# fperezgamonal/flownet2-tf

Measured on AMD Instinct MI355X. Metric: forward pairs/sec at 512x384 (FlowNet2), higher is better.
Workload: dtype f16x2 (split fp16 hi+lo operands, 3 fp16 MFMAs per product, fp32 accumulate); 1 GPU; FlowNet2 forward, batch=4 synthetic 512x384 pairs per GPU, seeded synthetic weights; pairs_per_gpu=4, parallelism=dp1 (no collective)

## Files before the change

### flownet2-tf_amd/csrc/conv.hip

```cpp
#include "conv_common.h"
#include <cstdlib>

namespace fn2 {

template <typename T, typename OutT, int TC, int WC, int WP>
__global__ void __launch_bounds__(256) conv_igemm_kernel(const ConvArgs p) {
  constexpr int CH = 16 / (int)sizeof(T);
  constexpr int BC = WC * TC * 16;
  constexpr int BP = WP * 64;
  constexpr int NT = 256;
  static_assert(WC * WP == 4, "4 waves per block");
  constexpr int NPR = BP / 64;
  constexpr int NWR = (BC * 4 + NT - 1) / NT;
  constexpr int WSWZ_BIT = (TC == 4) ? 5 : (TC == 2) ? 4 : 3;
  __shared__ uint4 lds[2][(BC + BP) * 4];

  const int tid = threadIdx.x, lane = tid & 63, wave = tid >> 6;
  const int wc = wave / WP, wp = wave % WP;
  const int cid = tid & 3;

  int pad_y = p.pad, pad_x = p.pad, oy_off = 0, ox_off = 0, osc = 1;
  const T* wgt = reinterpret_cast<const T*>(p.wgt);
  const int phase = blockIdx.z / p.splitk, split = blockIdx.z - phase * p.splitk;
  if (p.deconv) {
// ... 840 lines not shown
  FN2_REQUIRE(d->up_src == nullptr || ((d->kind == 1 || d->kind == 5) && d->up_w != nullptr && d->up_c0 >= 0 &&
                                       d->up_c0 + 2 <= d->out.cs && !d->accumulate),
              "conv2d: up_src rides on a kind-1 / kind-5 transposed conv (up_w set, [up_c0, up_c0 + 2) inside the out buffer)");
  FN2_REQUIRE(d->cin_pad % 8 == 0 && d->cin_pad >= d->in.c, "conv2d: cin_pad must be a multiple of 8 >= Cin");
  FN2_REQUIRE(d->in.cs % 8 == 0 && d->in.c0 % 8 == 0, "conv2d: input channel stride/offset must be multiples of 8");
  if (d->kind != 2)
    FN2_REQUIRE(d->in.c0 + d->cin_pad <= d->in.cs, "conv2d: padded input channels exceed the buffer stride");
  const int esz = dtype_size(d->in.dtype);
  const int CH = 16 / esz;
  FN2_REQUIRE(d->kpad > 0 && d->kpad % (4 * CH) == 0, "conv2d: kpad must be a multiple of one k-step");
  fn2_conv_plan plan;
  rc = fn2_conv2d_plan(d->in.dtype, d->cin_pad, d->out.c, &plan);
  if (rc) return rc;
  const bool wfrag = d->wgt_layout == 2;
  if (wfrag)
    FN2_REQUIRE(plan.layout == 1 && plan.cout_tile >= 64 && d->in.dtype == FN2_F16X2 && d->kind != 2,
                "conv2d: wgt_layout 2 (fragment order) is for split-fp16 layers with more than 32 output channels");
  else
    FN2_REQUIRE(d->wgt_layout == plan.layout, "conv2d: wgt_layout %d does not match fn2_conv2d_plan (%d)", d->wgt_layout,
                plan.layout);
  const int tile = plan.cout_tile;
  FN2_REQUIRE(d->cout_pad % tile == 0 && d->cout_pad >= d->out.c, "conv2d: cout_pad must be a multiple of the cout tile");
  FN2_REQUIRE(d->act == FN2_ACT_NONE || d->act == FN2_ACT_LEAKY, "conv2d: bad activation");
  FN2_REQUIRE(d->out.dtype == d->in.dtype || d->out.dtype == FN2_F32 ||
                  (d->in.dtype == FN2_F32 && d->out.dtype == FN2_F16X2),
              "conv2d: output dtype must be the input dtype, fp32, or split-fp16 from an fp32 stem");
  if (d->in.dtype == FN2_F16X2) FN2_REQUIRE(d->in.cs % 8 == 0 && d->in.c0 % 8 == 0, "conv2d: split-fp16 views are group (8) aligned");
  if (d->out.dtype == FN2_F16X2) FN2_REQUIRE(d->out.cs % 8 == 0 && d->out.c0 % 8 == 0, "conv2d: split-fp16 views are group (8) aligned");

  ConvArgs& a = *out;
  a = ConvArgs{};
  a.KH_KW_hint = 0;
// ... 16 lines not shown
  } else if (d->kind == 2) {
    FN2_REQUIRE(d->kh >= 1 && d->kw >= 1 && d->stride >= 1 && d->pad == 0, "stem conv: pad must be baked into the input buffer");
    FN2_REQUIRE(d->in.c0 == 0 && d->in.c == d->in.cs, "stem conv: the input view must be the whole buffer");
    FN2_REQUIRE(d->cin_pad >= d->kw * d->in.cs, "stem conv: run (cin_pad) shorter than kw*cs");
    FN2_REQUIRE(d->wgt_layout == 1, "stem conv: runs on the LDS-DMA kernel only (run must be whole 128-byte lines)");
    a.KH = d->kh; a.KW = 1; a.stride = d->stride; a.pad = 0;
    a.KH_KW_hint = d->kw;
    a.OH = (d->in.h - d->kh) / d->stride + 1;
    a.OW = (d->in.w - d->kw) / d->stride + 1;
    FN2_REQUIRE(a.OH >= 1 && a.OW >= 1, "stem conv: kernel does not fit");
    FN2_REQUIRE(d->out.h == a.OH && d->out.w == a.OW, "stem conv: output spatial size %dx%d != expected %dx%d",
                d->out.h, d->out.w, a.OH, a.OW);
    a.deconv = 0; a.ph_pad0 = a.ph_pad1 = 0;
  } else if (d->kind == 5) {
    FN2_REQUIRE(d->kh == 4 && d->kw == 4 && d->stride == 2, "deconv (kind 5): only k=4 s=2 crop 1");
    FN2_REQUIRE((d->out.c == 16 || d->out.c == 32) && d->in.dtype == FN2_F16X2 && d->wgt_layout == 1 && d->cout_pad == 2 * d->out.c,
                "deconv (kind 5): 16 or 32 output channels, split-fp16 input, cout_pad = 2 Cout");
    FN2_REQUIRE(d->in.w % 128 == 0, "deconv (kind 5): input width must be a multiple of 128 (halo kernel tiles)");
    a.KH = 2; a.KW = 3; a.stride = 1; a.pad = 0;
    a.OH = d->in.h; a.OW = d->in.w;
    FN2_REQUIRE(d->out.h == 2 * d->in.h && d->out.w == 2 * d->in.w, "deconv: output must be 2H x 2W");
    a.deconv = 1;
    a.ph_pad0 = 1; a.ph_pad1 = 0;
    phases = 2;
  } else if (d->kind == 1) {
    FN2_REQUIRE(d->kh == 4 && d->kw == 4 && d->stride == 2, "deconv: only k=4 s=2 crop 1 (flownet_s.py:53-63)");
    a.KH = 2; a.KW = 2; a.stride = 1; a.pad = 0;
    a.OH = d->in.h; a.OW = d->in.w;
    FN2_REQUIRE(d->out.h == 2 * d->in.h && d->out.w == 2 * d->in.w, "deconv: output must be 2H x 2W");
    a.deconv = 1;
    a.ph_pad0 = 1; a.ph_pad1 = 0;
// ... 163 lines not shown
    const int kper = cdiv(a.ksteps, sk);
    sk = cdiv(a.ksteps, kper);
    if (d->wgt_layout >= 1) sk = cdiv(a.ksteps / 2, cdiv(kper, 2));
  }
  return sk < 1 ? 1 : sk;
}

int fn2_conv2d_kernel_name(const fn2_conv_desc* d, char* name, int cap) {
  FN2_REQUIRE(name && cap > 0, "conv2d_kernel_name: no buffer");
  name[0] = 0;
  if (!d || d->wgt_layout < 1 || is_flow_head(d)) return FN2_OK;
  conv_name_sink() = ConvNameSink{name, cap};
  const int rc = fn2_conv2d(d, nullptr);
  conv_name_sink() = ConvNameSink{nullptr, 0};
  return rc;
}

int fn2_conv2d(const fn2_conv_desc* d, void* stream) {
  ConvArgs a;
  int tile, phases;
  int rc = build_args(d, &a, &tile, &phases);
  if (rc) return rc;
  hipStream_t s = (hipStream_t)stream;
  if (is_flow_head(d)) {
    int blocks = grid_for((long)a.M * 64, 256);
    if (d->in.dtype == FN2_F16X2 && a.M <= 4096 && !(a.dbg & 32768)) {
      a.dbg |= 16384;
      blocks = a.M;
    } else {
      a.dbg &= ~16384;
// ... 274 lines not shown
```

### flownet2-tf_amd/csrc/conv2.hip

```cpp
#include "conv_common.h"

#include <type_traits>
#include <algorithm>
#include <utility>

#ifndef FN2_X2_ORDER
#define FN2_X2_ORDER 0
#endif
#ifndef FN2_CONV_ABLATE
#define FN2_CONV_ABLATE 0
#endif
#ifndef FN2_SETPRIO
#define FN2_SETPRIO 1
#endif

namespace fn2 {

typedef __attribute__((address_space(3))) void* lptr_t;

constexpr unsigned kOobOffset = 0x80000000u;

typedef int v4i_t __attribute__((ext_vector_type(4)));
typedef unsigned u32x4_t __attribute__((ext_vector_type(4)));

__device__ __forceinline__ v4i_t make_rsrc(const void* base, int bytes) {
  const unsigned long long a = (unsigned long long)base;
  return v4i_t{(int)(a & 0xffffffffu), (int)((a >> 32) & 0xffffu), bytes, 0x00020000};
}

__device__ __forceinline__ void dma16(const v4i_t rsrc, const void* lds, unsigned voff, int soff) {
  const unsigned la = (unsigned)(unsigned long long)(lptr_t)lds;
  asm volatile("s_mov_b32 m0, %0\n\ts_nop 0\n\tbuffer_load_dwordx4 %1, %2, %3 offen lds"
               :: "s"(la), "v"(voff), "s"(rsrc), "s"(soff) : "memory");
}

__device__ __forceinline__ void h5_ring_pixel(const ConvArgs& p, long m) {
  const int lane = threadIdx.x & 63;
  const int H = p.OH, W = p.OW, ring = 2 * W + 2 * (H - 2);
  const int nitems = 25 * p.h5_groups;
  const size_t case_stride = (size_t)nitems * 16;
  const x2_t* in = reinterpret_cast<const x2_t*>(p.in);
  float* pf = reinterpret_cast<float*>(p.out);
  const int n = (int)(m / ring), r = (int)(m - (long)n * ring);
  int y, x;
  if (r < W) { y = 0; x = r; }
  else if (r < 2 * W) { y = H - 1; x = r - W; }
  else { const int q = r - 2 * W; y = 1 + (q >> 1); x = (q & 1) ? W - 1 : 0; }
  const int cy = y == 0 ? 0 : (y == H - 1 ? 2 : 1), cx = x == 0 ? 0 : (x == W - 1 ? 2 : 1);
// ... 195 lines not shown
          dma16(rsrc_w, &lds[(wave * (BC / 4) + i * 8) * 8], woff[i], ((ky * p.KW + kx) * spt + sc) * 128);
      }
    } else {
      constexpr int j = i - NWI;
      const unsigned tbit = (1u << ky) | (1u << (8 + kx));
      const int toff = ((ky * p.W + kx) * p.in_cs + sc * 8 * CH) * ESZ;
      const unsigned voff = ((vmask[j] & tbit) == tbit && wstage < kt1) ? (unsigned)(roff[j] + toff) : kOobOffset;
      if (!(FN2_CONV_ABLATE && (p.dbg & 1)))
        dma16(rsrc_x, &lds[(BOFF + wave * (BP / 4) + j * 8) * 8], voff, 0);
    }
  };
  u32x4_t wfa[WREG ? 4 : 1], wfb[WREG ? 4 : 1], wfc[(WREG && STAGES == 3) ? 4 : 1];
  const unsigned wlane = (unsigned)lane * 16u;
  const int wtile_off = WREG ? ((c0 >> 5) + wc) * (p.ksteps * 4096) : 0;
  auto load_w = [&](u32x4_t (&wf)[WREG ? 4 : 1]) {
    if constexpr (WREG) {
      const int soff = wtile_off + ((ky * p.KW + kx) * spt + sc) * 4096;
      asm volatile("buffer_load_dwordx4 %0, %4, %5, %6 offen\n\t"
                   "buffer_load_dwordx4 %1, %4, %5, %6 offen offset:1024\n\t"
                   "buffer_load_dwordx4 %2, %4, %5, %6 offen offset:2048\n\t"
                   "buffer_load_dwordx4 %3, %4, %5, %6 offen offset:3072"
                   : "=&v"(wf[0]), "=&v"(wf[1]), "=&v"(wf[2]), "=&v"(wf[3])
                   : "v"(wlane), "s"(rsrc_w), "s"(soff) : "memory");
    }
  };
  auto advance1 = [&]() {
    ++wstage;
    if (tap_outer) {
      if (++sc == spt) {
        sc = 0;
        if (++kx == kwi) { kx = 0; ++ky; }
      }
      if (ky == khi) { ky = 0; sc = spt; }
    } else if (++kx == kwi) {
      kx = 0;
      if (++ky == khi) { ky = 0; ++sc; }
    }
  };
  auto advance = [&]() {
// ... 2 lines not shown
  };
  auto issue_stage = [&](uint4* lds) {
    [&]<int... I>(std::integer_sequence<int, I...>) {
      (issue_piece(std::integral_constant<int, I>{}, lds), ...);
    }(std::make_integer_sequence<int, NWI + NPI>{});
    advance();
  };
  auto issue_stage_w = [&](uint4* lds, u32x4_t (&wf)[WREG ? 4 : 1]) {
    [&]<int... I>(std::integer_sequence<int, I...>) {
      (issue_piece(std::integral_constant<int, I>{}, lds), ...);
    }(std::make_integer_sequence<int, NWI + NPI>{});
    load_w(wf);
    advance();
  };
  auto wait_w = [&](u32x4_t (&wf)[WREG ? 4 : 1]) {
    if constexpr (WREG)
      asm volatile("s_waitcnt vmcnt(0)" : "+v"(wf[0]), "+v"(wf[1]), "+v"(wf[2]), "+v"(wf[3]) :: "memory");
  };

  const int fr = lane & 31, fh = lane >> 5, fsw = (fr >> 1) & 7;
  f32x16 acc[TCN][TPN];
#pragma unroll
  for (int tc = 0; tc < TCN; ++tc)
#pragma unroll
    for (int tp = 0; tp < TPN; ++tp)
#pragma unroll
      for (int q = 0; q < 16; ++q) acc[tc][tp][q] = 0.f;
  f32x4 acc16[M16 ? TCN * 2 : 1][M16 ? TPN * 2 : 1];
  if constexpr (M16) {
#pragma unroll
    for (int a = 0; a < TCN * 2; ++a)
#pragma unroll
// ... 452 lines not shown
  }
  if (wide) {
    const int rr = lane / CPR, ch = lane - rr * CPR;
    OutT* ob = out + p.out_c0 + c0 + wc * WCOLS + ch * 4;
#pragma unroll
    for (int i = 0; i < WROWS / RPI; ++i) {
      const int row = i * RPI + rr;
      const uint4 v = *reinterpret_cast<const uint4*>(tl + row * RS + ch * 4);
      const int opix = rowoff[row];
      if (opix >= 0) *reinterpret_cast<uint4*>(ob + (size_t)opix * p.out_cs) = v;
    }
  }
#endif
}

template <typename OutT, int WC, int WP, int TCN, int TPN, int KW>
__global__ void __launch_bounds__(256) conv_halo_kernel(const ConvArgs p) {
#if defined(__HIP_DEVICE_COMPILE__)
  using T = x2_t;
  constexpr int ESZ = 4;
  constexpr int BC = WC * TCN * 32, BP = WP * TPN * 32;
  static_assert(WC * WP == 4, "4 waves per block");
  constexpr int NWI = BC / 32;
  constexpr int BROWS = BP + 8;
  constexpr int NBP = BROWS / 8;
  constexpr int NBW = (NBP + 3) / 4;
  __shared__ uint4 ldsA[2][BC * 8];
  __shared__ uint4 ldsB[2][BROWS * 8];

  const int tid = threadIdx.x, lane = tid & 63;
  const int wave = __builtin_amdgcn_readfirstlane(tid >> 6);
  const int wc = wave / WP, wp = wave % WP;

  int pad_y = p.pad, pad_x = p.pad, oy_off = 0, ox_off = 0, osc = 1;
  const T* wgt = reinterpret_cast<const T*>(p.wgt);
  const int phase = blockIdx.z;
  const unsigned wrow_bytes = (unsigned)p.ksteps * 128u;
  if (p.merged) {
    pad_y = phase ? p.ph_pad1 : p.ph_pad0; pad_x = 1; oy_off = phase; ox_off = 0; osc = 2;
    wgt += (size_t)phase * p.cout_pad * (wrow_bytes / ESZ);
  } else if (p.deconv) {
    const int a = phase >> 1, b = phase & 1;
// ... 23 lines not shown
    const int row = wave * (BC / 4) + j * 8 + lrow;
    woff[j] = (unsigned)(c0 + row) * wrow_bytes + (unsigned)((lphys ^ ((row >> 1) & 7)) * 16);
  }
  int boff[NBW];
  bool bok[NBW];
#pragma unroll
  for (int j = 0; j < NBW; ++j) {
    const int q = wave + 4 * j;
    const int e = q * 8 + lrow;
    const int ix = ix_base + e;
    bok[j] = q < NBP && e < BP + KW - 1 && ix >= 0 && ix < p.W;
    boff[j] = (((tn * p.H + iy_base) * p.W + ix) * p.in_cs + p.in_c0) * ESZ + (lphys ^ ((e >> 1) & 7)) * 16;
  }
  const int spt = p.cin_chunks >> 3;
  const int nsup = spt * p.KH;
  auto issue_B = [&](int sup, uint4* lds) {
    const int sc = sup / p.KH, ky = sup - sc * p.KH;
    const bool yok = (unsigned)(iy_base + ky) < (unsigned)p.H;
    const int toff = (ky * p.W * p.in_cs) * ESZ + sc * 128;
#pragma unroll
    for (int j = 0; j < NBW; ++j) {
      const int q = wave + 4 * j;
      if (q < NBP) dma16(rsrc_x, &lds[q * 64], (bok[j] && yok) ? (unsigned)(boff[j] + toff) : kOobOffset, 0);
    }
  };
  auto issue_A = [&](int sup, int kx, uint4* lds) {
    const int sc = sup / p.KH, ky = sup - sc * p.KH;
    const int soff = ((ky * KW + kx) * spt + sc) * 128;
#pragma unroll
    for (int j = 0; j < NWI; ++j) dma16(rsrc_w, &lds[(wave * (BC / 4) + j * 8) * 8], woff[j], soff);
  };

  const int fr = lane & 31, fh = lane >> 5, fsw = (fr >> 1) & 7;
  f32x16 acc[TCN][TPN];
#pragma unroll
  for (int tc = 0; tc < TCN; ++tc)
#pragma unroll
    for (int tp = 0; tp < TPN; ++tp)
#pragma unroll
// ... 18 lines not shown
      }
#pragma unroll
      for (int tc = 0; tc < TCN; ++tc)
#pragma unroll
        for (int tp = 0; tp < TPN; ++tp) {
          acc[tc][tp] = mfma_32x32x16<f16_t>(al[tc], bh[tp], acc[tc][tp]);
          acc[tc][tp] = mfma_32x32x16<f16_t>(ah[tc], bl[tp], acc[tc][tp]);
          acc[tc][tp] = mfma_32x32x16<f16_t>(ah[tc], bh[tp], acc[tc][tp]);
        }
    }
#if FN2_SETPRIO
    __builtin_amdgcn_s_setprio(0);
#endif
  };

  issue_B(0, ldsB[0]);
  issue_A(0, 0, ldsA[0]);
  asm volatile("s_waitcnt vmcnt(0)" ::: "memory");
  __syncthreads();
  int abuf = 0;
  for (int sup = 0; sup < nsup; ++sup) {
#pragma unroll
    for (int kx = 0; kx < KW; ++kx) {
      if (kx + 1 < KW) issue_A(sup, kx + 1, ldsA[abuf ^ 1]);
      else if (sup + 1 < nsup) issue_A(sup + 1, 0, ldsA[abuf ^ 1]);
      if (kx == 0 && sup + 1 < nsup) issue_B(sup + 1, ldsB[(sup + 1) & 1]);
      compute(ldsA[abuf], ldsB[sup & 1], kx);
      asm volatile("s_waitcnt vmcnt(0)" ::: "memory");
      __syncthreads();
      abuf ^= 1;
    }
  }

  OutT* out = reinterpret_cast<OutT*>(p.out);
  const bool vec16 = (p.out_cs % 8 == 0) && (p.out_c0 % 8 == 0);
  constexpr int ERS = 36;
  static_assert(sizeof(ldsA) >= 4 * 32 * ERS * 4 || sizeof(ldsB) >= 4 * 32 * ERS * 4, "epilogue tiles fit a stage array");
  float* const etl = reinterpret_cast<float*>(sizeof(ldsA) >= 4 * 32 * ERS * 4 ? &ldsA[0][0] : &ldsB[0][0]) + wave * (32 * ERS);
#pragma unroll
  for (int tc = 0; tc < TCN; ++tc) {
    int cout_base = c0 + wc * TCN * 32 + tc * 32 + fh * 16;
    int bsel = 0;
    if (p.merged) { bsel = cout_base / p.Cout; cout_base -= bsel * p.Cout; if (bsel > 1) continue; }
    float bias[16];
#pragma unroll
// ... 510 lines not shown
    snprintf(conv_name_sink().buf, conv_name_sink().cap, "conv_stem_kernel<%s, %d>",
             is_x2<OutT>::value ? "fn2::x2_t" : "float", a.ksteps);
    return true;
  }
  switch (a.ksteps) {
    case 1: hipLaunchKernelGGL((conv_stem_kernel<OutT, 1>), dim3(blocks), dim3(256), 0, s, a, ntiles); break;
    case 2: hipLaunchKernelGGL((conv_stem_kernel<OutT, 2>), dim3(blocks), dim3(256), 0, s, a, ntiles); break;
    case 3: hipLaunchKernelGGL((conv_stem_kernel<OutT, 3>), dim3(blocks), dim3(256), 0, s, a, ntiles); break;
    default: hipLaunchKernelGGL((conv_stem_kernel<OutT, 4>), dim3(blocks), dim3(256), 0, s, a, ntiles); break;
  }
  return true;
}

template <typename OutT>
static bool launch_halo(const ConvArgs& a, int tile, int phases, hipStream_t s) {
  if (((a.dbg & 2048) && !a.merged) || a.stride != 1 || a.splitk != 1 || a.kg != 1 || !a.bp64 || a.wfrag || (a.KW != 2 && a.KW != 3)) return false;
  if (a.deconv && (a.kh_ph[0] != a.KH || a.kh_ph[1] != a.KH || a.kw_ph[0] != a.KW || a.kw_ph[1] != a.KW)) return false;
  if (tile == 128 && a.bp64 == 2 && !(a.dbg & 4096)) return false;
  if (a.bp64 == 3) return false;
  const int bp = tile == 128 ? 64 : 128;
  if (a.OW % bp != 0 || a.M % bp != 0) return false;
  dim3 block(256);
#define FN2_HALO(GY, ...)                                                                         \
  do {                                                                                            \
    dim3 grid(a.M / bp, GY, phases);                                                              \
    if (conv_name_sink().buf)                                                                     \
      snprintf(conv_name_sink().buf, conv_name_sink().cap, "conv_halo_kernel<%s, %s, %d>",       \
               is_x2<OutT>::value ? "fn2::x2_t" : "float", #__VA_ARGS__, a.KW);                    \
    else if (a.KW == 3) hipLaunchKernelGGL((conv_halo_kernel<OutT, __VA_ARGS__, 3>), grid, block, 0, s, a); \
    else hipLaunchKernelGGL((conv_halo_kernel<OutT, __VA_ARGS__, 2>), grid, block, 0, s, a);      \
  } while (0)
  if (tile == 128) FN2_HALO(a.cout_pad / 128, 2, 2, 2, 1);
  else if (tile == 64) FN2_HALO(a.cout_pad / 64, 1, 4, 2, 1);
  else FN2_HALO(a.cout_pad / 32, 1, 4, 1, 1);
#undef FN2_HALO
  return true;
}

template <typename T> static const char* type_name();
template <> const char* type_name<float>() { return "float"; }
template <> const char* type_name<bf16_t>() { return "__bf16"; }
template <> const char* type_name<f16_t>() { return "_Float16"; }
template <> const char* type_name<x2_t>() { return "fn2::x2_t"; }

ConvNameSink& conv_name_sink() {
  static thread_local ConvNameSink sink{nullptr, 0};
  return sink;
}

// ... 4 lines not shown
  const char* e_m16 = getenv("FN2_M16_MIN");
  const bool m16 = is_x2<T>::value && !(a.dbg & 512) &&
                   ((a.dbg & 1024) || (e_m16 && tile == 128 && a.bp64 == 1 && a.kg == 1 && a.splitk == 1 &&
                                       blocks64 >= atoi(e_m16)));
#define FN2_LAUNCH2(GX, GY, THREADS, ...)                                                              \
  do {                                                                                                 \
    dim3 grid(GX, GY, z);                                                                              \
    if (conv_name_sink().buf)                                                                          \
      snprintf(conv_name_sink().buf, conv_name_sink().cap, "conv_igemm2_kernel<%s, %s, %s, %s>", type_name<T>(), \
               type_name<OutT>(), #__VA_ARGS__, m16 ? "true" : "false");                              \
    else if (m16) hipLaunchKernelGGL((conv_igemm2_kernel<T, OutT, __VA_ARGS__, is_x2<T>::value>), grid, dim3(THREADS), 0, s, a); \
    else hipLaunchKernelGGL((conv_igemm2_kernel<T, OutT, __VA_ARGS__, false>), grid, dim3(THREADS), 0, s, a);            \
  } while (0)
  if (a.wfrag) {
    if constexpr (is_x2<T>::value) {
      if (tile == 64) {
        dim3 grid(cdiv(a.M, 128), a.cout_pad / 64, z);
        if (conv_name_sink().buf)
          snprintf(conv_name_sink().buf, conv_name_sink().cap, "conv_igemm2_kernel<%s, %s, 2, 2, 1, 2, 2, 1, false, true, %s>",
                   type_name<T>(), type_name<OutT>(), a.splitk > 1 ? "true" : "false");
        else if (a.splitk > 1)
          hipLaunchKernelGGL((conv_igemm2_kernel<T, OutT, 2, 2, 1, 2, 2, 1, false, true, true>), grid, dim3(256), 0, s, a);
        else
          hipLaunchKernelGGL((conv_igemm2_kernel<T, OutT, 2, 2, 1, 2, 2, 1, false, true, false>), grid, dim3(256), 0, s, a);
      } else {
        dim3 grid(cdiv(a.M, 64), a.cout_pad / 128, z);
        const bool slab = a.splitk > 1;
        ConvArgs ah = a;
        if (a.fh_M > 0 && slab && !conv_name_sink().buf) {
          const char* e = getenv("FN2_FH_BLOCKS");
          const long per_z = (long)grid.x * grid.y;
// ... 89 lines not shown
```

### flownet2-tf_amd/src/_hip.py

```python
import ctypes as C
import os

import numpy as np
import torch

_HERE = os.path.dirname(os.path.abspath(__file__))
LIB_PATH = os.path.join(os.path.dirname(_HERE), "lib", "libflownet2_hip.so")

FN2_F32, FN2_BF16, FN2_F16, FN2_F16X2 = 0, 1, 2, 3
ACT_NONE, ACT_LEAKY = 0, 1
OK = 0
ERR_INVALID_ARGUMENT, ERR_UNSUPPORTED, ERR_HIP = -1, -2, -3


class Fn2Tensor(C.Structure):
    _fields_ = [("data", C.c_void_p), ("dtype", C.c_int32), ("n", C.c_int32), ("h", C.c_int32),
                ("w", C.c_int32), ("c", C.c_int32), ("cs", C.c_int32), ("c0", C.c_int32)]


class Fn2ConvPlan(C.Structure):
    _fields_ = [("layout", C.c_int32), ("cout_tile", C.c_int32), ("kstep_elems", C.c_int32),
                ("wgt_dtype", C.c_int32)]


# ... 28 lines not shown
    "fn2_correlation_f32_ws": (_i, [_p, _p, _p] + [_i] * 9 + [_p, C.c_int64, _p]),
    "fn2_correlation_grad_f32": (_i, [_p] * 5 + [_i] * 9 + [_p]),
    "fn2_flow_warp_f32": (_i, [_p, _p, _p, _i, _i, _i, _i, _p]),
    "fn2_flow_warp_grad_f32": (_i, [_p] * 5 + [_i] * 4 + [_p]),
    "fn2_downsample_f32": (_i, [_p, _p] + [_i] * 6 + [_p]),
    "fn2_downsample_scaled_f32": (_i, [_p, _f, _p] + [_i] * 6 + [_p]),
    "fn2_fill_zero": (_i, [_p, C.c_int64, _p]),
    "fn2_add_f32": (_i, [_p, _p, C.c_int64, _p]),
    "fn2_slice_copy_f32": (_i, [_tp, _p, _p]),
    "fn2_resize_bilinear_f32": (_i, [_p, _p] + [_i] * 6 + [_f, _p]),
    "fn2_conv2d_plan": (_i, [_i, _i, _i, C.POINTER(Fn2ConvPlan)]),
    "fn2_conv2d_workspace_bytes": (C.c_int64, [C.POINTER(Fn2ConvDesc)]),
    "fn2_conv2d": (_i, [C.POINTER(Fn2ConvDesc), _p]),
    "fn2_conv2d_kernel_name": (_i, [C.POINTER(Fn2ConvDesc), C.c_char_p, _i]),
    "fn2_conv2d_splits": (_i, [C.POINTER(Fn2ConvDesc)]),
    "fn2_augment_f32": (_i, [_p, _p, _p, _p, _i, _i, _i, _i, _i, _i, _p]),
    "fn2_flow_augmentation_f32": (_i, [_p, _p, _p, _p, _i, _i, _i, _i, _i, _p]),
    "fn2_flow_head_gather": (_i, [_p, _i, _p, _p, _i, _i, _i, _p]),
    "fn2_upsample_flow": (_i, [_p, _p, _p, _tp, _i, _i, _i, _p]),
    "fn2_flow_head_tail": (_i, [_p, _i, _i, _p, _p, _i, _i, _i, _i, _p, _p, _tp, _p]),
    "fn2_flow_head_tail_slabs": (_i, [_p, _i, _i, C.c_int64, _f, _i, _p, _p, _i, _i, _i, _i, _p, _p, _tp, _p]),
    "fn2_flow_head_ring": (_i, [_tp, _p, _p, _p, _p]),
    "fn2_flow_head5": (_i, [_tp, _p, _i, _i, _f, _p, _p, _i, _p, _p, _p]),
    "fn2_u8_to_f32_lut": (_i, [_p, _p, _p, C.c_int64, _p]),
    "fn2_pack_pair": (_i, [_p, _p, _tp, _i, _p]),
    "fn2_pack_interp_u8": (_i, [_p, _p, _p, _p, _p, _tp, _i, _p]),
    "fn2_pack_image": (_i, [_p, _i, _tp, _i, _i, _p]),
    "fn2_pack_image_s2d": (_i, [_p, _i, _i, _i, _tp, _i, _i, _p]),
    "fn2_correlation_fused": (_i, [_tp, _tp, _tp, _i, _i, _i, _p]),
    "fn2_stack_input": (_i, [_p, _p, _p, _tp, _i, _p]),
# ... 115 lines not shown
```

### flownet2-tf_amd/src/engine.py

```python
import ctypes as C
import math
import os

import numpy as np
import torch

from . import _hip, netdefs, weights as W

_DT = {"f32": torch.float32, "bf16": torch.bfloat16, "f16": torch.float16, "f16x2": torch.float32}
_CODE = {"f32": _hip.FN2_F32, "bf16": _hip.FN2_BF16, "f16": _hip.FN2_F16, "f16x2": _hip.FN2_F16X2}
_TILE_ARGS = {128: "2, 2, 2, 2", 64: "1, 4, 2, 2", 32: "1, 4, 1, 2"}


def conv2_kernel_args(tile, m, cout_pad, phases, x2=True):
    dbg = int(os.environ.get("FN2_CONV_DBG", "0"))
    blocks64 = -(-m // 64) * (cout_pad // 128) * phases if tile == 128 else 0
    big = "FN2_M16_MIN" in os.environ and blocks64 >= max(int(os.environ["FN2_M16_MIN"]), 513)
    m16 = "true" if (x2 and not dbg & 512 and (dbg & 1024 or big)) else "false"
    full = dbg & 32
    if tile < 128:
        base = {64: "1, 4, 2, 2, 2, 1", 32: "1, 4, 1, 2, 2, 1"}[tile] if full else {64: "1, 4, 2, 1, 2, 1", 32: "1, 4, 1, 1, 2, 1"}[tile]
        return f"{base}, {m16}"
    blocks = -(-m // 64) * (cout_pad // 128) * phases
    if not full and int(os.environ.get("FN2_KG", "1")):
# ... 224 lines not shown
                out_scale = 2.0 ** (-k2)
        wdev = W.packed_to_device(packed, plan.wgt_dtype, self.device)
        d = _hip.Fn2ConvDesc()
        d.inp = self._v(sbuf, sc, sc0)
        d.out = self._v(dbuf, dc, dc0)
        d.wgt = wdev.data_ptr()
        d.bias = bias.data_ptr() if bias is not None else None
        d.kind = 0 if kind == "conv" else (5 if merged else 1)
        d.kh = d.kw = k
        d.stride, d.pad = stride, pad
        d.act = _hip.ACT_LEAKY if act else _hip.ACT_NONE
        d.cin_pad, d.cout_pad, d.kpad = cin_pad, cout_pad, kpad
        d.wgt_layout = layout
        d.out_scale = out_scale
        frag = False
        if (self.fragment_weights and layout == 1 and tile >= int(os.environ.get("FN2_WREG_TILE_MIN", "128"))
                and plan.wgt_dtype == _hip.FN2_F16X2 and self._wants_fragments(d)):
            wdev = W.to_fragment_order(wdev)
            d.wgt, d.wgt_layout, frag = wdev.data_ptr(), 2, True
        self.keep += [d, wdev, bias]
        self.conv_descs.append(d)
        self.desc_branch.append(self._branch)
        up_rec = None
        if self._pending_head is not None and kind != "conv":
            hd = self._pending_head
            assert up_after is not None and hd.inp.data == d.inp.data and hd.inp.c0 == d.inp.c0, (scope, name)
            d.head = C.addressof(hd)
            self._pending_head = None
        if up_after is not None:
            assert kind != "conv" and (not merged or cout == 16)
            up_name, up_src, (ubuf, uc0, uc) = up_after
            assert ubuf is dbuf and uc == 2
# ... 35 lines not shown
        need = int(self.lib.fn2_conv2d_workspace_bytes(C.byref(d)))
        if need <= 0 or not int(os.environ.get("FN2_HEAD_SLABS", "1")):
            return _hip.ptr(head_t), t_cs, 1, 0, 1.0
        ws = torch.empty((need + 3) // 4, dtype=torch.float32, device=self.device)
        d.workspace, d.workspace_bytes, d.raw_partials = ws.data_ptr(), need, 1
        self.keep.append(ws)
        self._own_ws.add(C.addressof(d))
        splits = int(self.lib.fn2_conv2d_splits(C.byref(d)))
        if splits <= 1:
            d.raw_partials = 0
            return _hip.ptr(head_t), t_cs, 1, 0, 1.0
        ws_cs = (d.out.c + 3) // 4 * 4
        return ws.data_ptr(), ws_cs, splits, d.out.n * d.out.h * d.out.w * ws_cs, float(d.out_scale) or 1.0

    def _wants_fragments(self, d):
        need = int(self.lib.fn2_conv2d_workspace_bytes(C.byref(d)))
        d.workspace, d.workspace_bytes = (1, need) if need else (None, 0)
        buf = C.create_string_buffer(256)
        rc = self.lib.fn2_conv2d_kernel_name(C.byref(d), buf, 256)
        d.workspace, d.workspace_bytes = None, 0
        which = os.environ.get("FN2_WREG_KERNELS", "false>")
        return rc == 0 and buf.value.decode().startswith("conv_igemm2_kernel") and buf.value.decode().endswith(which)

    def _head_gemm(self, scope, spec, src, dst, up=None):
        name, kind, k, stride, pad, cin, cout, act = spec
        sbuf, sc0, sc = src
        pf = dst[0]
        in_code = self._code(sbuf)
        esz = 2 if in_code in (_hip.FN2_BF16, _hip.FN2_F16) else 4
        cin_line = _round_up(cin, 128 // esz)
        if sc0 + cin_line > sbuf.shape[3]:
            return False
        plan = _hip.conv_plan(in_code, cin_line, 18)
        if plan.layout != 1:
            return False
        w = np.asarray(self._w(f"{scope}/{name}/weights"), np.float32)
        w1 = np.ascontiguousarray(w.transpose(2, 0, 1, 3)).reshape(1, 1, cin, 18)
# ... 700 lines not shown
```

### include/flownet2_hip.h

```cpp
#ifndef FLOWNET2_HIP_H_
#define FLOWNET2_HIP_H_

#include <stddef.h>
#include <stdint.h>

#ifdef __cplusplus
extern "C" {
#endif

typedef enum {
  FN2_OK = 0,
  FN2_ERR_INVALID_ARGUMENT = -1,
  FN2_ERR_UNSUPPORTED = -2,
  FN2_ERR_HIP = -3
} fn2_status;

typedef enum { FN2_F32 = 0, FN2_BF16 = 1, FN2_F16 = 2, FN2_F16X2 = 3 } fn2_dtype;

typedef enum { FN2_ACT_NONE = 0, FN2_ACT_LEAKY = 1  } fn2_act;

typedef struct {
  void* data;
  int32_t dtype;
  int32_t n, h, w;
// ... 62 lines not shown
  const float* up_src;
  const float* up_w;
  const float* up_bias;
  int32_t up_c0;
  const void* head;
  int32_t raw_partials;
} fn2_conv_desc;

typedef struct {
  int32_t layout, cout_tile, kstep_elems, wgt_dtype;
} fn2_conv_plan;
int fn2_conv2d_plan(int in_dtype, int cin_pad, int cout, fn2_conv_plan* plan);
int64_t fn2_conv2d_workspace_bytes(const fn2_conv_desc* d);
int fn2_conv2d(const fn2_conv_desc* d, void* stream);
int fn2_conv2d_kernel_name(const fn2_conv_desc* desc, char* name, int cap);
int fn2_conv2d_splits(const fn2_conv_desc* desc);

int fn2_flow_head_gather(const float* t, int t_cs, const float* bias, float* out, int n, int h, int w, void* stream);
int fn2_flow_head_tail(const float* t, int t_cs, int taps, const float* bias, float* pf, int n, int h, int w, int ring,
                       const float* up_w, const float* up_bias, const fn2_tensor* up_out, void* stream);
int fn2_flow_head_tail_slabs(const float* t, int t_cs, int nslab, int64_t slab_stride, float scale, int taps, const float* bias,
                             float* pf, int n, int h, int w, int ring, const float* up_w, const float* up_bias,
                             const fn2_tensor* up_out, void* stream);
int fn2_flow_head5(const fn2_tensor* x, const void* wgt, int cin_pad, int kpad, float out_scale, const float* bias, float* pf,
                   int ring, const float* ring_w, const float* ring_b, void* stream);
int fn2_flow_head_ring(const fn2_tensor* x, const float* wc, const float* bc, float* pf, void* stream);
int fn2_upsample_flow(const float* in, const float* w, const float* bias, const fn2_tensor* out, int n, int h, int wd,
                      void* stream);

int fn2_u8_to_f32_lut(const unsigned char* src, const float* lut256, float* dst, long count, void* stream);
// ... 77 lines not shown
```

Measured before the change: 1101 pairs/s.

## Stream fragment-order weights into registers in the halo conv kernel

Adds a WFRAG variant of the halo convolution kernel that loads pre-swizzled weight fragments directly from global memory into registers. This skips the LDS staging of weights, drops the A-side LDS buffers and interleaves the per-kx weight loads with the pixel DMA and MFMA work. The fragment-weight decision moves into C (fn2_conv2d_wants_fragments) and now also covers 32-cout and 128-cout halo layers. The risk is more register pressure and vmcnt ordering that depends on a fixed count of DMA pieces per wave.

```diff
diff --git a/flownet2-tf_amd/csrc/conv.hip b/flownet2-tf_amd/csrc/conv.hip
--- a/flownet2-tf_amd/csrc/conv.hip
+++ b/flownet2-tf_amd/csrc/conv.hip
@@ -1,5 +1,6 @@
 #include "conv_common.h"
 #include <cstdlib>
+#include <cstring>
 
 namespace fn2 {
 
@@ -878,8 +879,8 @@
   if (rc) return rc;
   const bool wfrag = d->wgt_layout == 2;
   if (wfrag)
-    FN2_REQUIRE(plan.layout == 1 && plan.cout_tile >= 64 && d->in.dtype == FN2_F16X2 && d->kind != 2,
-                "conv2d: wgt_layout 2 (fragment order) is for split-fp16 layers with more than 32 output channels");
+    FN2_REQUIRE(plan.layout == 1 && plan.cout_tile >= 32 && d->in.dtype == FN2_F16X2 && d->kind != 2,
+                "conv2d: wgt_layout 2 (fragment order) is for split-fp16 layers on the LDS-DMA tiles, stems excluded");
   else
     FN2_REQUIRE(d->wgt_layout == plan.layout, "conv2d: wgt_layout %d does not match fn2_conv2d_plan (%d)", d->wgt_layout,
                 plan.layout);
@@ -926,7 +927,7 @@
     a.deconv = 0; a.ph_pad0 = a.ph_pad1 = 0;
   } else if (d->kind == 5) {
     FN2_REQUIRE(d->kh == 4 && d->kw == 4 && d->stride == 2, "deconv (kind 5): only k=4 s=2 crop 1");
-    FN2_REQUIRE((d->out.c == 16 || d->out.c == 32) && d->in.dtype == FN2_F16X2 && d->wgt_layout == 1 && d->cout_pad == 2 * d->out.c,
+    FN2_REQUIRE((d->out.c == 16 || d->out.c == 32) && d->in.dtype == FN2_F16X2 && d->wgt_layout >= 1 && d->cout_pad == 2 * d->out.c,
                 "deconv (kind 5): 16 or 32 output channels, split-fp16 input, cout_pad = 2 Cout");
     FN2_REQUIRE(d->in.w % 128 == 0, "deconv (kind 5): input width must be a multiple of 128 (halo kernel tiles)");
     a.KH = 2; a.KW = 3; a.stride = 1; a.pad = 0;
@@ -1120,6 +1121,35 @@
   const int rc = fn2_conv2d(d, nullptr);
   conv_name_sink() = ConvNameSink{nullptr, 0};
   return rc;
+}
+
+int fn2_conv2d_wants_fragments(const fn2_conv_desc* d) {
+  if (!d || d->wgt_layout != 1 || d->in.dtype != FN2_F16X2 || d->kind == 2 || is_flow_head(d)) return 0;
+  fn2_conv_desc q = *d;
+  const int64_t need = fn2_conv2d_workspace_bytes(&q);
+  q.workspace = need > 0 ? reinterpret_cast<void*>(1) : nullptr;
+  q.workspace_bytes = need;
+  char n1[256], n2[256];
+  fn2_conv2d_kernel_name(&q, n1, sizeof n1);
+  const size_t l1 = strlen(n1);
+  fn2_conv_plan plan;
+  if (fn2_conv2d_plan(d->in.dtype, d->cin_pad, d->out.c, &plan) != FN2_OK) return 0;
+  const char* e_min = getenv("FN2_WREG_TILE_MIN");
+  const bool igemm_ok = plan.cout_tile >= (e_min ? atoi(e_min) : 128);
+  if (strncmp(n1, "conv_igemm2_kernel", 18) == 0) {
+    const char* e_sfx = getenv("FN2_WREG_KERNELS");
+    const char* sfx = e_sfx ? e_sfx : "false>";
+    const size_t ls = strlen(sfx);
+    return igemm_ok && l1 >= ls && strcmp(n1 + l1 - ls, sfx) == 0;
+  }
+  if (strncmp(n1, "conv_halo_kernel", 16) == 0) {
+    q.wgt_layout = 2;
+    fn2_conv2d_kernel_name(&q, n2, sizeof n2);
+    const size_t l2 = strlen(n2);
+    if (strncmp(n2, "conv_halo_kernel", 16) == 0) return l2 >= 6 && strcmp(n2 + l2 - 6, " true>") == 0;
+    return igemm_ok && strncmp(n2, "conv_igemm2_kernel", 18) == 0;
+  }
+  return 0;
 }
 
 int fn2_conv2d(const fn2_conv_desc* d, void* stream) {
diff --git a/flownet2-tf_amd/csrc/conv2.hip b/flownet2-tf_amd/csrc/conv2.hip
--- a/flownet2-tf_amd/csrc/conv2.hip
+++ b/flownet2-tf_amd/csrc/conv2.hip
@@ -32,6 +32,19 @@
   const unsigned la = (unsigned)(unsigned long long)(lptr_t)lds;
   asm volatile("s_mov_b32 m0, %0\n\ts_nop 0\n\tbuffer_load_dwordx4 %1, %2, %3 offen lds"
                :: "s"(la), "v"(voff), "s"(rsrc), "s"(soff) : "memory");
+}
+
+__device__ __forceinline__ void load_wfrag(u32x4_t (&wf)[4], const v4i_t rsrc, unsigned wlane, int soff) {
+  asm volatile("buffer_load_dwordx4 %0, %4, %5, %6 offen\n\t"
+               "buffer_load_dwordx4 %1, %4, %5, %6 offen offset:1024\n\t"
+               "buffer_load_dwordx4 %2, %4, %5, %6 offen offset:2048\n\t"
+               "buffer_load_dwordx4 %3, %4, %5, %6 offen offset:3072"
+               : "=&v"(wf[0]), "=&v"(wf[1]), "=&v"(wf[2]), "=&v"(wf[3])
+               : "v"(wlane), "s"(rsrc), "s"(soff) : "memory");
+}
+template <int N>
+__device__ __forceinline__ void wait_wfrag(u32x4_t (&wf)[4]) {
+  asm volatile("s_waitcnt vmcnt(%4)" : "+v"(wf[0]), "+v"(wf[1]), "+v"(wf[2]), "+v"(wf[3]) : "n"(N) : "memory");
 }
 
 __device__ __forceinline__ void h5_ring_pixel(const ConvArgs& p, long m) {
@@ -257,15 +270,7 @@
   const unsigned wlane = (unsigned)lane * 16u;
   const int wtile_off = WREG ? ((c0 >> 5) + wc) * (p.ksteps * 4096) : 0;
   auto load_w = [&](u32x4_t (&wf)[WREG ? 4 : 1]) {
-    if constexpr (WREG) {
-      const int soff = wtile_off + ((ky * p.KW + kx) * spt + sc) * 4096;
-      asm volatile("buffer_load_dwordx4 %0, %4, %5, %6 offen\n\t"
-                   "buffer_load_dwordx4 %1, %4, %5, %6 offen offset:1024\n\t"
-                   "buffer_load_dwordx4 %2, %4, %5, %6 offen offset:2048\n\t"
-                   "buffer_load_dwordx4 %3, %4, %5, %6 offen offset:3072"
-                   : "=&v"(wf[0]), "=&v"(wf[1]), "=&v"(wf[2]), "=&v"(wf[3])
-                   : "v"(wlane), "s"(rsrc_w), "s"(soff) : "memory");
-    }
+    if constexpr (WREG) load_wfrag(wf, rsrc_w, wlane, wtile_off + ((ky * p.KW + kx) * spt + sc) * 4096);
   };
   auto advance1 = [&]() {
     ++wstage;
@@ -298,8 +303,7 @@
     advance();
   };
   auto wait_w = [&](u32x4_t (&wf)[WREG ? 4 : 1]) {
-    if constexpr (WREG)
-      asm volatile("s_waitcnt vmcnt(0)" : "+v"(wf[0]), "+v"(wf[1]), "+v"(wf[2]), "+v"(wf[3]) :: "memory");
+    if constexpr (WREG) wait_wfrag<0>(wf);
   };
 
   const int fr = lane & 31, fh = lane >> 5, fsw = (fr >> 1) & 7;
@@ -782,18 +786,19 @@
 #endif
 }
 
-template <typename OutT, int WC, int WP, int TCN, int TPN, int KW>
+template <typename OutT, int WC, int WP, int TCN, int TPN, int KW, bool WFRAG = false>
 __global__ void __launch_bounds__(256) conv_halo_kernel(const ConvArgs p) {
 #if defined(__HIP_DEVICE_COMPILE__)
   using T = x2_t;
   constexpr int ESZ = 4;
   constexpr int BC = WC * TCN * 32, BP = WP * TPN * 32;
   static_assert(WC * WP == 4, "4 waves per block");
+  static_assert(!WFRAG || TCN == 1, "WFRAG: one 32-cout tile per wave");
   constexpr int NWI = BC / 32;
   constexpr int BROWS = BP + 8;
   constexpr int NBP = BROWS / 8;
   constexpr int NBW = (NBP + 3) / 4;
-  __shared__ uint4 ldsA[2][BC * 8];
+  __shared__ uint4 ldsA[WFRAG ? 1 : 2][WFRAG ? 1 : BC * 8];
   __shared__ uint4 ldsB[2][BROWS * 8];
 
   const int tid = threadIdx.x, lane = tid & 63;
@@ -847,15 +852,18 @@
   }
   const int spt = p.cin_chunks >> 3;
   const int nsup = spt * p.KH;
-  auto issue_B = [&](int sup, uint4* lds) {
+  auto issue_B_part = [&](int sup, uint4* lds, auto j0_c, auto j1_c) {
     const int sc = sup / p.KH, ky = sup - sc * p.KH;
-    const bool yok = (unsigned)(iy_base + ky) < (unsigned)p.H;
+    const bool yok = (unsigned)(iy_base + ky) < (unsigned)p.H && sup < nsup;
     const int toff = (ky * p.W * p.in_cs) * ESZ + sc * 128;
 #pragma unroll
-    for (int j = 0; j < NBW; ++j) {
+    for (int j = decltype(j0_c)::value; j < decltype(j1_c)::value; ++j) {
       const int q = wave + 4 * j;
       if (q < NBP) dma16(rsrc_x, &lds[q * 64], (bok[j] && yok) ? (unsigned)(boff[j] + toff) : kOobOffset, 0);
     }
+  };
+  auto issue_B = [&](int sup, uint4* lds) {
+    issue_B_part(sup, lds, std::integral_constant<int, 0>{}, std::integral_constant<int, NBW>{});
   };
   auto issue_A = [&](int sup, int kx, uint4* lds) {
     const int sc = sup / p.KH, ky = sup - sc * p.KH;
@@ -904,21 +912,85 @@
 #endif
   };
 
-  issue_B(0, ldsB[0]);
-  issue_A(0, 0, ldsA[0]);
-  asm volatile("s_waitcnt vmcnt(0)" ::: "memory");
-  __syncthreads();
-  int abuf = 0;
-  for (int sup = 0; sup < nsup; ++sup) {
-#pragma unroll
-    for (int kx = 0; kx < KW; ++kx) {
-      if (kx + 1 < KW) issue_A(sup, kx + 1, ldsA[abuf ^ 1]);
-      else if (sup + 1 < nsup) issue_A(sup + 1, 0, ldsA[abuf ^ 1]);
-      if (kx == 0 && sup + 1 < nsup) issue_B(sup + 1, ldsB[(sup + 1) & 1]);
-      compute(ldsA[abuf], ldsB[sup & 1], kx);
-      asm volatile("s_waitcnt vmcnt(0)" ::: "memory");
+  if constexpr (WFRAG) {
+    u32x4_t wf[KW][4];
+    const unsigned wlane = (unsigned)lane * 16u;
+    const int wtile_off = ((c0 >> 5) + wc) * (p.ksteps * 4096);
+    auto load_w = [&](int tb, int kx, u32x4_t (&f)[4]) { load_wfrag(f, rsrc_w, wlane, wtile_off + (tb + kx * spt) * 4096); };
+    auto compute_w = [&](const u32x4_t (&f)[4], const uint4* lb, int kx) {
+#if FN2_SETPRIO
+      __builtin_amdgcn_s_setprio(1);
+#endif
+#pragma unroll
+      for (int q = 0; q < 2; ++q) {
+        uint4 bh[TPN], bl[TPN];
+#pragma unroll
+        for (int t = 0; t < TPN; ++t) {
+          const int rb = wp * TPN * 32 + t * 32 + fr + kx, sw = (rb >> 1) & 7;
+          bh[t] = lb[rb * 8 + ((4 * q + 2 * fh) ^ sw)];
+          bl[t] = lb[rb * 8 + ((4 * q + 2 * fh + 1) ^ sw)];
+        }
+        const uint4 ah = __builtin_bit_cast(uint4, f[2 * q]), al = __builtin_bit_cast(uint4, f[2 * q + 1]);
+#pragma unroll
+        for (int tp = 0; tp < TPN; ++tp) {
+          acc[0][tp] = mfma_32x32x16<f16_t>(al, bh[tp], acc[0][tp]);
+          acc[0][tp] = mfma_32x32x16<f16_t>(ah, bl[tp], acc[0][tp]);
+          acc[0][tp] = mfma_32x32x16<f16_t>(ah, bh[tp], acc[0][tp]);
+        }
+      }
+#if FN2_SETPRIO
+      __builtin_amdgcn_s_setprio(0);
+#endif
+    };
+    static_assert(NBP % 4 == 1, "wave 0 issues NBW pixel pieces per super-stage, the others NBW - 1 (vmcnt literal below)");
+    constexpr std::integral_constant<int, 0> kJ0{};
+    constexpr std::integral_constant<int, NBW - 1> kJlast{};
+    constexpr std::integral_constant<int, NBW> kJend{};
+    load_w(0, 0, wf[0]);
+    issue_B(0, ldsB[0]);
+    wait_wfrag<0>(wf[0]);
+    __syncthreads();
+    int ky = 0, sc = 0;
+    for (int sup = 0; sup < nsup; ++sup) {
+      const uint4* lb = ldsB[sup & 1];
+      const int tb = ky * KW * spt + sc;
+      if (++ky == p.KH) { ky = 0; ++sc; }
+      const int tb1 = ky * KW * spt + sc;
+      issue_B_part(sup + 1, ldsB[(sup + 1) & 1], kJlast, kJend);
+      load_w(tb, 1, wf[1]);
+      issue_B_part(sup + 1, ldsB[(sup + 1) & 1], kJ0, kJlast);
+      compute_w(wf[0], lb, 0);
+      wait_wfrag<NBW - 1>(wf[1]);
+      if constexpr (KW == 3) {
+        load_w(tb, 2, wf[2]);
+        compute_w(wf[1], lb, 1);
+        wait_wfrag<0>(wf[2]);
+        load_w(tb1, 0, wf[0]);
+        compute_w(wf[2], lb, 2);
+      } else {
+        load_w(tb1, 0, wf[0]);
+        compute_w(wf[1], lb, 1);
+      }
+      wait_wfrag<0>(wf[0]);
       __syncthreads();
-      abuf ^= 1;
+    }
+  } else {
+    issue_B(0, ldsB[0]);
+    issue_A(0, 0, ldsA[0]);
+    asm volatile("s_waitcnt vmcnt(0)" ::: "memory");
+    __syncthreads();
+    int abuf = 0;
+    for (int sup = 0; sup < nsup; ++sup) {
+#pragma unroll
+      for (int kx = 0; kx < KW; ++kx) {
+        if (kx + 1 < KW) issue_A(sup, kx + 1, ldsA[abuf ^ 1]);
+        else if (sup + 1 < nsup) issue_A(sup + 1, 0, ldsA[abuf ^ 1]);
+        if (kx == 0 && sup + 1 < nsup) issue_B(sup + 1, ldsB[(sup + 1) & 1]);
+        compute(ldsA[abuf], ldsB[sup & 1], kx);
+        asm volatile("s_waitcnt vmcnt(0)" ::: "memory");
+        __syncthreads();
+        abuf ^= 1;
+      }
     }
   }
 
@@ -1459,10 +1531,11 @@
 
 template <typename OutT>
 static bool launch_halo(const ConvArgs& a, int tile, int phases, hipStream_t s) {
-  if (((a.dbg & 2048) && !a.merged) || a.stride != 1 || a.splitk != 1 || a.kg != 1 || !a.bp64 || a.wfrag || (a.KW != 2 && a.KW != 3)) return false;
+  if (((a.dbg & 2048) && !a.merged) || a.stride != 1 || a.splitk != 1 || a.kg != 1 || !a.bp64 || (a.KW != 2 && a.KW != 3)) return false;
   if (a.deconv && (a.kh_ph[0] != a.KH || a.kh_ph[1] != a.KH || a.kw_ph[0] != a.KW || a.kw_ph[1] != a.KW)) return false;
-  if (tile == 128 && a.bp64 == 2 && !(a.dbg & 4096)) return false;
+  if (tile == 128 && (a.wfrag ? a.wfrag == 2 : a.bp64 == 2) && !(a.dbg & 4096)) return false;
   if (a.bp64 == 3) return false;
+  if (a.wfrag && (tile == 64 || (tile == 32 && a.KW != 3))) return false;
   const int bp = tile == 128 ? 64 : 128;
   if (a.OW % bp != 0 || a.M % bp != 0) return false;
   dim3 block(256);
@@ -1475,9 +1548,26 @@
     else if (a.KW == 3) hipLaunchKernelGGL((conv_halo_kernel<OutT, __VA_ARGS__, 3>), grid, block, 0, s, a); \
     else hipLaunchKernelGGL((conv_halo_kernel<OutT, __VA_ARGS__, 2>), grid, block, 0, s, a);      \
   } while (0)
-  if (tile == 128) FN2_HALO(a.cout_pad / 128, 2, 2, 2, 1);
+#define FN2_HALO_W(GY, ...)                                                                       \
+  do {                                                                                            \
+    dim3 grid(a.M / bp, GY, phases);                                                              \
+    if (conv_name_sink().buf)                                                                     \
+      snprintf(conv_name_sink().buf, conv_name_sink().cap, "conv_halo_kernel<%s, %s, %d, true>", \
+               is_x2<OutT>::value ? "fn2::x2_t" : "float", #__VA_ARGS__, a.KW);                    \
+    else if (a.KW == 3) hipLaunchKernelGGL((conv_halo_kernel<OutT, __VA_ARGS__, 3, true>), grid, block, 0, s, a); \
+    else hipLaunchKernelGGL((conv_halo_kernel<OutT, __VA_ARGS__, 2, true>), grid, block, 0, s, a); \
+  } while (0)
+  if (a.wfrag && tile == 128) FN2_HALO_W(a.cout_pad / 128, 4, 1, 1, 2);
+  else if (a.wfrag) {
+    dim3 grid(a.M / bp, a.cout_pad / 32, phases);
+    if (conv_name_sink().buf)
+      snprintf(conv_name_sink().buf, conv_name_sink().cap, "conv_halo_kernel<%s, 1, 4, 1, 1, 3, true>", is_x2<OutT>::value ? "fn2::x2_t" : "float");
+    else hipLaunchKernelGGL((conv_halo_kernel<OutT, 1, 4, 1, 1, 3, true>), grid, block, 0, s, a);
+  }
+  else if (tile == 128) FN2_HALO(a.cout_pad / 128, 2, 2, 2, 1);
   else if (tile == 64) FN2_HALO(a.cout_pad / 64, 1, 4, 2, 1);
   else FN2_HALO(a.cout_pad / 32, 1, 4, 1, 1);
+#undef FN2_HALO_W
 #undef FN2_HALO
   return true;
 }
@@ -1512,7 +1602,9 @@
   } while (0)
   if (a.wfrag) {
     if constexpr (is_x2<T>::value) {
-      if (tile == 64) {
+      if (tile == 32) {
+        return fail(FN2_ERR_UNSUPPORTED, "conv fast path: fragment-order weights on the 32-cout tile need the halo kernel");
+      } else if (tile == 64) {
         dim3 grid(cdiv(a.M, 128), a.cout_pad / 64, z);
         if (conv_name_sink().buf)
           snprintf(conv_name_sink().buf, conv_name_sink().cap, "conv_igemm2_kernel<%s, %s, 2, 2, 1, 2, 2, 1, false, true, %s>",
diff --git a/flownet2-tf_amd/src/_hip.py b/flownet2-tf_amd/src/_hip.py
--- a/flownet2-tf_amd/src/_hip.py
+++ b/flownet2-tf_amd/src/_hip.py
@@ -66,6 +66,7 @@
     "fn2_conv2d": (_i, [C.POINTER(Fn2ConvDesc), _p]),
     "fn2_conv2d_kernel_name": (_i, [C.POINTER(Fn2ConvDesc), C.c_char_p, _i]),
     "fn2_conv2d_splits": (_i, [C.POINTER(Fn2ConvDesc)]),
+    "fn2_conv2d_wants_fragments": (_i, [C.POINTER(Fn2ConvDesc)]),
     "fn2_augment_f32": (_i, [_p, _p, _p, _p, _i, _i, _i, _i, _i, _i, _p]),
     "fn2_flow_augmentation_f32": (_i, [_p, _p, _p, _p, _i, _i, _i, _i, _i, _p]),
     "fn2_flow_head_gather": (_i, [_p, _i, _p, _p, _i, _i, _i, _p]),
diff --git a/flownet2-tf_amd/src/engine.py b/flownet2-tf_amd/src/engine.py
--- a/flownet2-tf_amd/src/engine.py
+++ b/flownet2-tf_amd/src/engine.py
@@ -262,8 +262,7 @@
         d.wgt_layout = layout
         d.out_scale = out_scale
         frag = False
-        if (self.fragment_weights and layout == 1 and tile >= int(os.environ.get("FN2_WREG_TILE_MIN", "128"))
-                and plan.wgt_dtype == _hip.FN2_F16X2 and self._wants_fragments(d)):
+        if self.fragment_weights and layout == 1 and plan.wgt_dtype == _hip.FN2_F16X2 and self._wants_fragments(d):
             wdev = W.to_fragment_order(wdev)
             d.wgt, d.wgt_layout, frag = wdev.data_ptr(), 2, True
         self.keep += [d, wdev, bias]
@@ -329,13 +328,7 @@
         return ws.data_ptr(), ws_cs, splits, d.out.n * d.out.h * d.out.w * ws_cs, float(d.out_scale) or 1.0
 
     def _wants_fragments(self, d):
-        need = int(self.lib.fn2_conv2d_workspace_bytes(C.byref(d)))
-        d.workspace, d.workspace_bytes = (1, need) if need else (None, 0)
-        buf = C.create_string_buffer(256)
-        rc = self.lib.fn2_conv2d_kernel_name(C.byref(d), buf, 256)
-        d.workspace, d.workspace_bytes = None, 0
-        which = os.environ.get("FN2_WREG_KERNELS", "false>")
-        return rc == 0 and buf.value.decode().startswith("conv_igemm2_kernel") and buf.value.decode().endswith(which)
+        return bool(self.lib.fn2_conv2d_wants_fragments(C.byref(d)))
 
     def _head_gemm(self, scope, spec, src, dst, up=None):
         name, kind, k, stride, pad, cin, cout, act = spec
diff --git a/include/flownet2_hip.h b/include/flownet2_hip.h
--- a/include/flownet2_hip.h
+++ b/include/flownet2_hip.h
@@ -100,6 +100,7 @@
 int64_t fn2_conv2d_workspace_bytes(const fn2_conv_desc* d);
 int fn2_conv2d(const fn2_conv_desc* d, void* stream);
 int fn2_conv2d_kernel_name(const fn2_conv_desc* desc, char* name, int cap);
+int fn2_conv2d_wants_fragments(const fn2_conv_desc* desc);
 int fn2_conv2d_splits(const fn2_conv_desc* desc);
 
 int fn2_flow_head_gather(const float* t, int t_cs, const float* bias, float* out, int n, int h, int w, void* stream);
```

Result: no change. 1106 pairs/s, median of 6 (+0.4%).
